# spdes/chirpgp

Measured on AMD Instinct MI355X. Metric: filter+smoother trial-steps/s (batch x T / wall), higher is better.
Workload: dtype f64; 1 GPU; C2: discrete EKF+EKS (demos/ekfs_mle.py model); d=4, T=10000, batch_per_gpu=1000, global_batch=1000, parallelism=trials sharded x1

## Files before the change

### chirpgp_amd/csrc/cgp_mfma4.hpp

```cpp
#pragma once
#include "cgp_coop4.hpp"

namespace cgp {


CGP_DEV double mfma4(double a, double b, double c) { return __builtin_amdgcn_mfma_f64_4x4x4f64(a, b, c, 0, 0, 0); }

constexpr int kCheckedChunks = 16;

struct Ekf4MfmaConst {
    double M0, M1, M2, M3, rho, ang;
    double Hr, Xi, Sig;
    double kc, ks, kj, kk;
    double SigHq, c0;
    double kcr, ksr, kja;
    double angm;
    double pa, pb, pA0, pB0, m1, m2;
    CGP_DEV void fold() { kcr = kc * rho; ksr = ks * rho; kja = kj * ang; angm = (kc != 0.0 || ks != 0.0) ? ang : 0.0; }
    CGP_DEV void fold_e1(int r, int q) {
        fold();
        angm = q == 0 ? ang : (q == 1 ? -ang : 0.0);
        pa = q < 2 ? rho : 0.0;
        pb = q == 0 ? -rho : (q == 1 ? rho : 0.0);
        pA0 = q == 2 ? M0 : (q == 3 ? M3 : 0.0);
        pB0 = q == 2 ? M1 : (q == 3 ? M2 : 0.0);
        m1 = r == q ? 1.0 : 0.0;
        m2 = r == (q ^ 1) ? 1.0 : 0.0;
    }
    template <bool E1> CGP_DEV void load(const HarmonicLCD<1>& model, const FilterIO& io, int64_t trial, int r, int q) {
        M0 = model.M[0]; M1 = model.M[1]; M2 = model.M[2]; M3 = model.M[3];
        rho = model.rho;
        ang = (model.dt * kTwoPi) * model.fs;
        Hr = io.H[trial * io.H_stride + r];
        Xi = io.Xi[trial * io.Xi_stride];
        Sig = lane_sigma_entry(model, r, q);
        const double mq = model.q;
        SigHq = (q == 1) ? mq : 0.0;
        c0 = mq + Xi;
        kc = ((q == 0 && r == 0) || (q == 1 && r == 1)) ? 1.0 : 0.0;
        ks = (q == 0 && r == 1) ? -1.0 : ((q == 1 && r == 0) ? 1.0 : 0.0);
        kj = (r == 2 && q == 0) ? -1.0 : ((r == 2 && q == 1) ? 1.0 : 0.0);
        kk = (q == 2) ? (r == 2 ? M0 : (r == 3 ? M1 : 0.0)) : ((q == 3) ? (r == 2 ? M2 : (r == 3 ? M3 : 0.0)) : 0.0);
        if constexpr (E1) fold_e1(r, q);
        else fold();
    }
};
struct Ekf4State {
    double P, ur, uq;
    CGP_DEV double u2() const { return dpp_f64<kQuadBcast2>(uq); }
    CGP_DEV double u2_replicated() const { return row_bcast_f64<2>(uq); }
    template <bool E1> CGP_DEV void load(const FilterIO& io, int64_t trial, int r, int q) {
        const double* __restrict__ m0p = io.m0 + trial * io.m0_stride;
        ur = E1 ? 0.0 : m0p[r]; uq = m0p[q];
        P = coop4_load_sym_entry(io.P0 + trial * io.P0_stride, r, q);
    }
};

template <int E1 = 0, bool GAPS = false>
CGP_DEV void ekf4_mfma_finish_j(const Ekf4MfmaConst& K, double y, double A, double B2, double kjd, Ekf4State& x, double& S, double& innov) {
    double J0T, f_r, f_q;
    if constexpr (E1 != 0) {
        f_q = fma(A, x.uq, B2 * dpp_f64<kQuadSwap1>(x.uq));
        J0T = fma(K.m1, A, K.m2 * B2);
        f_r = 0.0;
    } else {
        J0T = A;
        f_r = mfma4(J0T, x.ur, 0.0); f_q = mfma4(x.ur, J0T, 0.0);
    }
    const double RJT = fma(kjd, dpp_f64<kQuadSwap1>(f_q), J0T);
    double Pp, PHr, PHq;
    if constexpr (E1 != 0) {
        auto bcast1 = [](double v) { if constexpr (E1 == 2) return row_bcast_f64<1>(v); else return dpp_f64<kQuadBcast1>(v); };
        const double Q = mfma4(x.P, RJT, 0.0);
        const double Pa = bcast1(Q);
        PHq = mfma4(Pa, RJT, K.SigHq);
        Pp = mfma4(RJT, Q, K.Sig);
        PHr = bcast1(Pp);
        if constexpr (E1 == 1) {
            const double a = dpp_f64<kQuadBcast1>(RJT);
            S = mfma4(a, Pa, K.c0);
        } else {
            S = bcast1(PHq) + K.Xi;
        }
        innov = y - bcast1(f_q);
    } else {
        const double Q = mfma4(x.P, RJT, 0.0);
        Pp = mfma4(RJT, Q, K.Sig);
        PHr = mfma4(Pp, K.Hr, 0.0);
        PHq = mfma4(K.Hr, Pp, 0.0);
        S = mfma4(K.Hr, PHr, K.Xi);
        innov = y - mfma4(K.Hr, f_r, 0.0);
    }
    double rS = rcp_nr1(S), dy = innov;
    if constexpr (GAPS) {
        const bool gap = is_missing(y);
        rS = gap ? 0.0 : rS;
        dy = gap ? 0.0 : innov;
    }
    x.P = fma(-(PHr * rS), PHq, Pp);
    const double g = rS * dy;
    if constexpr (E1 == 0) x.ur = fma(PHr, g, f_r);
    x.uq = fma(PHq, g, f_q);
}
template <int E1 = 0, bool GAPS = false>
CGP_DEV void ekf4_mfma_finish(const Ekf4MfmaConst& K, double y, double c1, double s1, double dsp, Ekf4State& x, double& S, double& innov) {
    if constexpr (E1 != 0) {
        ekf4_mfma_finish_j<E1, GAPS>(K, y, fma(K.pa, c1, K.pA0), fma(K.pb, s1, K.pB0), K.kja * dsp, x, S, innov);
    } else {
        const double J0T = fma(K.kcr, c1, fma(K.ksr, s1, K.kk));
        ekf4_mfma_finish_j<E1, GAPS>(K, y, J0T, 0.0, K.kja * dsp, x, S, innov);
    }
}

template <int E1 = 0, bool GAPS = false>
CGP_DEV void ekf4_mfma_step_wide(const Ekf4MfmaConst& K, const WideRegs& W, double y, Ekf4State& x, double& S, double& innov, bool& bad) {
    double sp, dsp, s1, c1;
    bool ok1, ok2;
    softplus_pair_any(W, x.u2(), sp, dsp, ok1);
    fast_sincos_spec(W, K.ang * sp, s1, c1, ok2);
    bad = bad || !(ok1 && ok2);
    ekf4_mfma_finish<E1, GAPS>(K, y, c1, s1, dsp, x, S, innov);
}

template <int E1 = 0, bool GAPS = false>
CGP_DEV void ekf4_mfma_step_checked(const Ekf4MfmaConst& K, double y, Ekf4State& x, double& S, double& innov) {
    double sp, dsp, s1, c1;
    softplus_pair_uniform(x.u2(), sp, dsp);
    fast_sincos_uniform(K.ang * sp, s1, c1);
    ekf4_mfma_finish<E1, GAPS>(K, y, c1, s1, dsp, x, S, innov);
}

struct Ekf4Anchor {
    double th, A, B;
    template <int E1 = 0>
    CGP_DEV void set(const Ekf4MfmaConst& K, double sp, double c1, double s1) {
        th = K.angm * sp;
        if constexpr (E1 != 0) {
            A = fma(K.pa, c1, K.pA0);
            B = fma(K.pb, s1, K.pB0);
        } else {
            A = fma(K.kcr, c1, fma(K.ksr, s1, K.kk));
            B = fma(K.ksr, c1, -(K.kcr * s1));
        }
    }
};

template <int E1 = 0>
CGP_DEV void ekf4_anchor(const Ekf4MfmaConst& K, double u2, Ekf4Anchor& a) {
    double sp, dsp, s1, c1;
    softplus_pair_uniform(u2, sp, dsp);
    fast_sincos_uniform(K.ang * sp, s1, c1);
    a.template set<E1>(K, sp, c1, s1);
}

constexpr unsigned kIncrementBound = 0x3F780000u;
constexpr int kRegCommon = 0, kRegHigh = 1, kRegLow = 2, kRegAny = 3, kRegMid = 4;
struct Ekf4Verdict {
    unsigned u = 0u, umin = 0xFFFFFFFFu, d = 0u;
    int di = 0;
    bool any_bad = false;
    unsigned uabs = 0u;
    template <int REG = kRegCommon> CGP_DEV bool state_in_regime() const {
        if constexpr (REG == kRegAny) return !any_bad;
        if constexpr (REG == kRegMid) return uabs < 0x40000000u;
        if constexpr (REG == kRegLow) return umin >= 0xBFF80000u && u <= 0xC085DFFFu;
        constexpr unsigned lo = REG == kRegHigh ? 0x40140000u : 0x3FF80000u;
        return u <= 0x4085DFFFu && umin >= lo;
    }
    template <int REG = kRegCommon> CGP_DEV unsigned code() const {
        const bool state = __builtin_amdgcn_ballot_w64(!state_in_regime<REG>()) != 0;
        const bool jump = __builtin_amdgcn_ballot_w64((d & 0x7FFFFFFFu) >= kIncrementBound || ((unsigned)di & 0x7FFFFFFFu) >= kIncrementBound) != 0;
        return (state ? 1u : 0u) | (jump ? 2u : 0u);
    }
    template <int REG = kRegCommon> CGP_DEV unsigned long long uncommon() const {
        return __builtin_amdgcn_ballot_w64(!state_in_regime<REG>()) |
               __builtin_amdgcn_ballot_w64((d & 0x7FFFFFFFu) >= kIncrementBound || ((unsigned)di & 0x7FFFFFFFu) >= kIncrementBound);
    }
};
template <int E1, int REG = kRegCommon>
CGP_DEV void ekf4_mfma_step_spec1(const Ekf4MfmaConst& K, const SpecRegs& R, const SpecRegsHigh& RH, double y, Ekf4State& x, Ekf4Anchor& a,
                                  double& S, double& innov, Ekf4Verdict& verdict, const SpecRegsMid* RM = nullptr, const WideRegs* RW = nullptr) {
    const double u2 = (E1 == 2) ? x.u2_replicated() : x.u2();
    constexpr bool HIGH = REG == kRegHigh, LOW = REG == kRegLow, ANY = REG == kRegAny, MID = REG == kRegMid;
    double d, jfac;
    if constexpr (MID) {
        double ga, hj;
        softplus_mid_polys(*RM, u2, ga, hj);
        d = ga + fma(0.5 * K.angm, u2, -a.th);
        jfac = fma(u2, hj, 0.5 * K.kja);
    } else if constexpr (ANY) {
        double sp, dspf; bool ok;
        if (RW) softplus_pair_any(*RW, u2, sp, dspf, ok);
        else softplus_pair_any(u2, sp, dspf, ok);
        verdict.any_bad = verdict.any_bad || !ok;
        d = fma(K.angm, sp, -a.th);
        jfac = K.kja * dspf;
    } else {
        const double t = HIGH ? exp_neg_high(R, RH, u2) : exp_neg_lean1(R, LOW ? -u2 : u2);
        const double lin = LOW ? -a.th : fma(K.angm, u2, -a.th);
        double qa, dsp;
        if constexpr (HIGH) softplus_tail_high(RH, t, qa, dsp);
        else softplus_tail_lean(R, t, qa, dsp);
        d = fma(qa, t, lin);
        jfac = HIGH ? dsp : LOW ? (K.kja * t) * dsp : K.kja * dsp;
    }
    const double d2 = d * d;
    const double tau = d * fma(d2, R.c4, 0.5);
    const double sn = d * fma(d2, R.s3, 1.0);
    const double A1 = fma(tau, a.B, a.A);
    const double B = fma(-sn, A1, a.B);
    const double A = fma(tau, B, A1);
    const unsigned hx = (unsigned)__double2hiint(u2), hd = (unsigned)__double2hiint(d);
    if constexpr (MID) {
        const unsigned ha = hx & 0x7FFFFFFFu;
        verdict.uabs = verdict.uabs > ha ? verdict.uabs : ha;
    } else if constexpr (!ANY) {
        verdict.u = verdict.u > hx ? verdict.u : hx;
        verdict.umin = verdict.umin < hx ? verdict.umin : hx;
    }
    verdict.d = verdict.d > hd ? verdict.d : hd;
    verdict.di = verdict.di > (int)hd ? verdict.di : (int)hd;
    a.th += d; a.A = A; a.B = B;
    ekf4_mfma_finish_j<E1>(K, y, A, B, jfac, x, S, innov);
}

constexpr int kEkf4Unroll = 4;
constexpr int kEkf4FastGroups = 4;

#ifdef CGP_EKF4_KERNELS
template <bool E1>
CGP_DEV void ekf4_mfma_trial(const FilterIO& io, const ModelArgs& ma) {
    const int lane = threadIdx.x;
    const int r = lane >> 4, q = lane & 3;
    const FilterSpan span = filter_span(io, blockIdx.x);
    using Seg = SegRecord<4>;
    const int64_t trial = span.trial;

    HarmonicLCD<1> model;
    model.setup(ma.params + trial * ma.param_stride, ma.dt, ma.model_id);
    Ekf4MfmaConst K;
    K.template load<E1>(model, io, trial, r, q);
    Ekf4State x;
    x.template load<E1>(io, trial, r, q);
    const double* __restrict__ ys = io.record(trial);
    Tile4FilterOut out;
    out.init(io, trial, lane);
    const unsigned p_off = out.offP, m_off = out.offm;
    const bool nll_final = (io.flags & CGP_NLL_FINAL_ONLY) != 0;
    double* __restrict__ nll = (io.nll && !nll_final) ? io.nll + trial * io.T : nullptr;
    const bool want_nll = io.nll != nullptr;

    SpecRegs R;
    R.init(K.angm);
    SpecRegsHigh RH;
    RH.init(K.angm, K.kja);
    constexpr int kParkStride = 2;
    __shared__ double2 park[64 * kParkStride];
    __shared__ double ybuf[64 + 16];
    __shared__ double parkS[64], parkI[64];
    double cum = 0.0;
    int checked_left = 0, spec_off = 0, jump_streak = 0, spec_score = -4;
    unsigned n_high = 0, n_common = 0, n_redo = 0, n_checked = 0, n_high_left = 0, n_wide = 0, n_low = 0, n_mid = 0;
    Ekf4Anchor anchor_live;
    int anchor_age = -1;
    const int64_t Te = span.t_end;
    double ynext = (span.t_begin + lane < Te) ? ys[span.t_begin + lane] : 0.0;
    for (int64_t t0 = span.t_begin; t0 < Te; t0 += 64) {
        wave_lds_fence();
        const bool burn = t0 < span.t_out;
        const OobWindow Pw = out.P_window(burn), mw = out.m_window(burn);
        if (span.state && span.seg > 0 && t0 == span.t_out) {
            Seg::put_mean(span.state, Seg::kJunction, lane < 4, lane, x.uq);
            Seg::put_cov(span.state, Seg::kJunction, ((lane >> 2) & 3) == 0, r, q, x.P);
        }
        double ychunk = ynext;
        asm volatile("" : "+v"(ychunk));
        ynext = (t0 + 64 + lane < Te) ? ys[t0 + 64 + lane] : 0.0;
        const int nsteps = (Te - t0 < 64) ? (int)(Te - t0) : 64;
        const Ekf4State x0 = x;
        const unsigned hx0 = (unsigned)__builtin_amdgcn_readfirstlane(__double2hiint(x.u2()));
        const bool low = !nll_final && hx0 - 0xBFFC0000u <= 0xC085DFFFu - 0xBFFC0000u;
        const bool mid = !nll_final && (hx0 & 0x7FFFFFFFu) < 0x3FF80000u;
        const bool edge = !nll_final && !mid && (hx0 & 0x7FFFFFFFu) < 0x3FFC0000u;
        ybuf[lane] = ychunk;
        wave_lds_fence();
        Ekf4Anchor anchor0, anchor_end;
        const bool spec_allowed = spec_off == 0;
        if (!spec_allowed) anchor0 = anchor_live;
        else if (anchor_age < 0 || anchor_age >= 4) { ekf4_anchor<E1 ? 2 : 0>(K, x.u2(), anchor0); anchor_age = 0; }
        else anchor0 = anchor_live;
        auto chunk = [&](auto reg_c) {
            constexpr int REG = decltype(reg_c)::value;
            SpecRegsMid RM;
            if constexpr (REG == kRegMid) RM.init(K.angm, K.kja);
            WideRegs RW;
            if constexpr (REG == kRegAny) RW.init();
            Ekf4Anchor anchor = anchor0;
            Ekf4Verdict verdict;
            auto one = [&](int slot, unsigned k, double y) {
                double S, innov;
                ekf4_mfma_step_spec1<E1 ? 2 : 0, REG>(K, R, RH, y, x, anchor, S, innov, verdict, &RM, REG == kRegAny ? &RW : nullptr);
                park[(slot + k) * kParkStride] = make_double2(S, innov);
                const unsigned t = (unsigned)(t0 + slot);
                Pw.store_s(x.P, p_off + k * 128u, t * 128u);
                mw.store_s(x.uq, m_off + k * 32u, t * 32u);
            };
            int slot = 0;
            double2 ya = *reinterpret_cast<const double2*>(ybuf), yb = *reinterpret_cast<const double2*>(ybuf + 2);
            double2 yc = *reinterpret_cast<const double2*>(ybuf + 4), yd = *reinterpret_cast<const double2*>(ybuf + 6);
            for (; slot + 8 <= nsteps; slot += 8) {
                const double2 na = *reinterpret_cast<const double2*>(ybuf + slot + 8), nb = *reinterpret_cast<const double2*>(ybuf + slot + 10);
                const double2 nc = *reinterpret_cast<const double2*>(ybuf + slot + 12), nd = *reinterpret_cast<const double2*>(ybuf + slot + 14);
                one(slot, 0u, ya.x); one(slot, 1u, ya.y); one(slot, 2u, yb.x); one(slot, 3u, yb.y);
                one(slot, 4u, yc.x); one(slot, 5u, yc.y); one(slot, 6u, yd.x); one(slot, 7u, yd.y);
                ya = na; yb = nb; yc = nc; yd = nd;
            }
            for (; slot + 4 <= nsteps; slot += 4) {
                const double2 na = *reinterpret_cast<const double2*>(ybuf + slot + 4), nb = *reinterpret_cast<const double2*>(ybuf + slot + 6);
                one(slot, 0u, ya.x); one(slot, 1u, ya.y); one(slot, 2u, yb.x); one(slot, 3u, yb.y);
                ya = na; yb = nb;
            }
            for (; slot < nsteps; slot++) one(slot, 0u, readlane_f64(ychunk, slot));
            anchor_end = anchor;
            return verdict.template code<REG>();
        };
        unsigned uncommon = 1;
        int kept_reg = -1;
        const bool lean_tried = spec_allowed && (low || mid || (checked_left == 0 && !edge));
        if (lean_tried) {
            bool high = false;
            if constexpr (E1) high = !nll_final && hx0 - 0x401A0000u < 0x4085DFFFu - 0x401A0000u;
            if (low) {
                uncommon = chunk(std::integral_constant<int, kRegLow>{});
                if (uncommon == 0) n_low++;
            } else if (mid) {
                uncommon = chunk(std::integral_constant<int, kRegMid>{});
                if (uncommon == 0) n_mid++;
            } else {
                if (high) {
                    uncommon = chunk(std::integral_constant<int, kRegHigh>{});
                    if (uncommon != 0) { x = x0; n_high_left++; } else { n_high++; kept_reg = kRegHigh; }
                }
                if (uncommon != 0) {
                    uncommon = chunk(std::integral_constant<int, kRegCommon>{});
                    if (uncommon == 0) { n_common++; kept_reg = kRegCommon; }
                }
            }
        }
        if (uncommon != 0) {
            if (lean_tried) { x = x0; checked_left = (!(low || mid) && (uncommon & 1u)) ? kCheckedChunks : 1; n_redo++; }
            auto jumped = [&]() { jump_streak = jump_streak < 4 ? jump_streak + 1 : 4; if (spec_off < (1 << jump_streak)) spec_off = 1 << jump_streak; };
            auto failed = [&]() {
                spec_score = spec_score > -14 ? spec_score - 2 : -16;
                if (spec_score <= -8 && spec_off < 32) spec_off = 32;
                if (t0 == span.t_begin && spec_off < 8) spec_off = 8;
            };
            if (lean_tried) { failed(); if ((uncommon & 2u) != 0) jumped(); }
            if (spec_allowed && spec_off == 0) {
                uncommon = chunk(std::integral_constant<int, kRegAny>{});
                if (uncommon == 0) { if (!lean_tried) n_wide++; }
                else { failed(); if ((uncommon & 2u) != 0) jumped(); }
            }
        }
        if (uncommon == 0) {
            anchor_live = anchor_end; anchor_age++;
            if (jump_streak > 0) jump_streak--;
            if (spec_score < 8) spec_score++;
            if (checked_left > 0) checked_left--;
        } else {
            if (!spec_allowed) spec_off--;
            anchor_age = -1;
            x = x0;
            const bool redo = lean_tried;
            bool bad = false;
            WideRegs W;
            W.init();
            auto wide_one = [&](int slot, double y) {
                double S, innov;
                ekf4_mfma_step_wide<E1 ? 2 : 0>(K, W, y, x, S, innov, bad);
                park[slot * kParkStride] = make_double2(S, innov);
                const unsigned t = (unsigned)(t0 + slot);
                Pw.store_s(x.P, p_off, t * 128u);
                mw.store_s(x.uq, m_off, t * 32u);
            };
            int wslot = 0;
            for (; wslot + 4 <= nsteps; wslot += 4) {
                const double2 ya = *reinterpret_cast<const double2*>(ybuf + wslot), yb = *reinterpret_cast<const double2*>(ybuf + wslot + 2);
                wide_one(wslot, ya.x); wide_one(wslot + 1, ya.y); wide_one(wslot + 2, yb.x); wide_one(wslot + 3, yb.y);
            }
            for (; wslot < nsteps; wslot++) wide_one(wslot, readlane_f64(ychunk, wslot));
            if (__builtin_amdgcn_ballot_w64(bad) != 0) {
                x = x0;
                for (int slot = 0; slot < nsteps; slot++) {
                    double S, innov;
                    ekf4_mfma_step_checked<E1 ? 2 : 0>(K, readlane_f64(ychunk, slot), x, S, innov);
                    park[slot * kParkStride] = make_double2(S, innov);
                    const unsigned t = (unsigned)(t0 + slot);
                    Pw.store_s(x.P, p_off, t * 128u);
                    mw.store_s(x.uq, m_off, t * 32u);
                }
                if (!redo) n_checked++;
            } else if (!redo) n_wide++;
            if (checked_left > 0) checked_left--;
        }
        if (want_nll && !burn) {
            wave_lds_fence();
            const double2 si = park[(lane < nsteps ? lane : 0) * kParkStride];
            cum = nll_flush_wave(si.x, si.y, lane, nsteps, cum, nll ? nll + t0 : nullptr);
        }
        if (kept_reg >= 0 && checked_left == 0 && spec_off == 0 && t0 >= span.t_out) {
            auto fast_run = [&](auto reg_c) {
                constexpr int REG = decltype(reg_c)::value;
                for (;;) {
                    const int64_t t1 = t0 + 64;
                    if (t1 + 64 > Te) break;
                    const unsigned hx1 = (unsigned)__builtin_amdgcn_readfirstlane(__double2hiint(x.u2()));
                    const bool low1 = !nll_final && hx1 - 0xBFFC0000u <= 0xC085DFFFu - 0xBFFC0000u;
                    const bool mid1 = !nll_final && (hx1 & 0x7FFFFFFFu) < 0x3FF80000u;
                    const bool edge1 = !nll_final && !mid1 && (hx1 & 0x7FFFFFFFu) < 0x3FFC0000u;
                    bool high1 = false;
                    if constexpr (E1) high1 = !nll_final && hx1 - 0x401A0000u < 0x4085DFFFu - 0x401A0000u;
                    if (low1 || mid1 || edge1 || high1 != (REG == kRegHigh)) break;
                    wave_lds_fence();
                    double ychunk = ynext;
                    asm volatile("" : "+v"(ychunk));
                    ynext = (t1 + 64 + lane < Te) ? ys[t1 + 64 + lane] : 0.0;
                    const Ekf4State x1 = x;
                    ybuf[lane] = ychunk;
                    wave_lds_fence();
                    const bool reanchor = anchor_age >= 4;
                    Ekf4Anchor anchor;
                    if (reanchor) ekf4_anchor<E1 ? 2 : 0>(K, x.u2(), anchor);
                    else anchor = anchor_live;
                    Ekf4Verdict verdict;
                    auto one = [&](int slot, unsigned k, double y) {
                        double S, innov;
                        ekf4_mfma_step_spec1<E1 ? 2 : 0, REG>(K, R, RH, y, x, anchor, S, innov, verdict);
                        parkS[slot + k] = S; parkI[slot + k] = innov;
                        const unsigned t = (unsigned)(t1 + slot);
                        out.wP.store_s(x.P, p_off + k * 128u, t * 128u);
                        out.wm.store_s(x.uq, m_off + k * 32u, t * 32u);
                    };
                    double2 ya = *reinterpret_cast<const double2*>(ybuf), yb = *reinterpret_cast<const double2*>(ybuf + 2);
                    double2 yc = *reinterpret_cast<const double2*>(ybuf + 4), yd = *reinterpret_cast<const double2*>(ybuf + 6);
                    auto group8 = [&](int slot) {
                        const double2 na = *reinterpret_cast<const double2*>(ybuf + slot + 8), nb = *reinterpret_cast<const double2*>(ybuf + slot + 10);
                        const double2 nc = *reinterpret_cast<const double2*>(ybuf + slot + 12), nd = *reinterpret_cast<const double2*>(ybuf + slot + 14);
                        one(slot, 0u, ya.x); one(slot, 1u, ya.y); one(slot, 2u, yb.x); one(slot, 3u, yb.y);
                        one(slot, 4u, yc.x); one(slot, 5u, yc.y); one(slot, 6u, yd.x); one(slot, 7u, yd.y);
                        ya = na; yb = nb; yc = nc; yd = nd;
                    };
#pragma unroll 1
                    for (int slot = 0; slot < 64; slot += 8 * kEkf4FastGroups) {
#pragma unroll
                        for (int g = 0; g < kEkf4FastGroups; g++) group8(slot + 8 * g);
                    }
                    if (verdict.template code<REG>() != 0) { x = x1; ynext = ychunk; break; }
                    t0 = t1;
                    anchor_live = anchor; anchor_age = reanchor ? 1 : anchor_age + 1;
                    if (jump_streak > 0) jump_streak--;
                    if (spec_score < 8) spec_score++;
                    if constexpr (REG == kRegHigh) n_high++;
                    else n_common++;
                    if (want_nll) {
                        wave_lds_fence();
                        const double2 si = make_double2(parkS[lane], parkI[lane]);
                        cum = nll_flush_wave(si.x, si.y, lane, 64, cum, nll ? nll + t1 : nullptr);
                    }
                }
            };
            if (E1 && kept_reg == kRegHigh) { if constexpr (E1) fast_run(std::integral_constant<int, kRegHigh>{}); }
            else fast_run(std::integral_constant<int, kRegCommon>{});
        }
    }
    if (span.state) {
        Seg::put_mean(span.state, Seg::kEnd, lane < 4, lane, x.uq);
        Seg::put_cov(span.state, Seg::kEnd, ((lane >> 2) & 3) == 0, r, q, x.P);
        Seg::put_nll(span.state, lane, cum);
    } else if (lane == 0 && io.nll && nll_final) io.nll[trial] = cum;
    if (io.counters && lane == 0) {
        atomicAdd(io.counters + 0, (unsigned long long)n_high); atomicAdd(io.counters + 1, (unsigned long long)n_common);
        atomicAdd(io.counters + 2, (unsigned long long)n_redo); atomicAdd(io.counters + 3, (unsigned long long)n_checked);
        atomicAdd(io.counters + 4, (unsigned long long)n_high_left); atomicAdd(io.counters + 5, (unsigned long long)n_wide);
        atomicAdd(io.counters + 6, (unsigned long long)n_low); atomicAdd(io.counters + 7, (unsigned long long)n_mid);
    }
}

template <bool E1>
CGP_DEV void kf4_mfma_trial(const FilterIO& io, const ModelArgs& ma) {
    const int lane = threadIdx.x;
    const int r = lane >> 4, q = lane & 3;
    const int64_t trial = blockIdx.x;
    const double* __restrict__ prm = ma.params + trial * ma.param_stride;
    const double JT = prm[q * 4 + r];
    const double Sig = prm[16 + r * 4 + q];
    const double* __restrict__ Hp = io.H + trial * io.H_stride;
    const double Hr = Hp[r];
    const double Xi = io.Xi[trial * io.Xi_stride];

    const double* __restrict__ m0p = io.m0 + trial * io.m0_stride;
    double ur = m0p[r], uq = m0p[q];
    double P = coop4_load_sym_entry(io.P0 + trial * io.P0_stride, r, q);

    const int64_t T = io.T;
    const double* __restrict__ ys = io.record(trial);
    Tile4FilterOut out;
    out.init(io, trial, lane);

    __shared__ double2 park[64];
    __shared__ double ybuf[64 + 8];
    double cum = 0.0;
    double ynext = (lane < T) ? ys[lane] : 0.0;
    for (int64_t t0 = 0; t0 < T; t0 += 64) {
        double ychunk = ynext;
        asm volatile("" : "+v"(ychunk));
        ynext = (t0 + 64 + lane < T) ? ys[t0 + 64 + lane] : 0.0;
        const int nsteps = (T - t0 < 64) ? (int)(T - t0) : 64;
        wave_lds_fence();
        auto one = [&](int slot, double y) {
            const double f_r = mfma4(JT, ur, 0.0), f_q = mfma4(ur, JT, 0.0);
            const double Q = mfma4(P, JT, 0.0);
            double Pp, PHr, PHq, S, innov;
            if constexpr (E1) {
                Pp = mfma4(JT, Q, Sig);
                PHq = mfma4(Hr, Pp, 0.0);
                PHr = dpp_f64<kQuadBcast1>(Pp);
                S = dpp_f64<kQuadBcast1>(PHq) + Xi;
                innov = y - dpp_f64<kQuadBcast1>(f_q);
            } else {
                Pp = mfma4(JT, Q, Sig);
                PHr = mfma4(Pp, Hr, 0.0);
                PHq = mfma4(Hr, Pp, 0.0);
                S = mfma4(Hr, PHr, Xi);
                innov = y - mfma4(Hr, f_r, 0.0);
            }
            const double rS = rcp_nr1(S);
            P = fma(-(PHr * rS), PHq, Pp);
            const double g = rS * innov;
            ur = fma(PHr, g, f_r);
            uq = fma(PHq, g, f_q);
            park[slot] = make_double2(S, innov);
            const unsigned t = (unsigned)(t0 + slot);
            out.wP.store_s(P, out.offP, t * 128u);
            out.wm.store_s(uq, out.offm, t * 32u);
        };
        ybuf[lane] = ychunk;
        wave_lds_fence();
        int slot = 0;
        double2 ya = *reinterpret_cast<const double2*>(ybuf), yb = *reinterpret_cast<const double2*>(ybuf + 2);
        for (; slot + 4 <= nsteps; slot += 4) {
            const double2 na = *reinterpret_cast<const double2*>(ybuf + slot + 4), nb = *reinterpret_cast<const double2*>(ybuf + slot + 6);
            one(slot, ya.x); one(slot + 1, ya.y); one(slot + 2, yb.x); one(slot + 3, yb.y);
            ya = na; yb = nb;
        }
        for (; slot < nsteps; slot++) one(slot, readlane_f64(ychunk, slot));
        if (out.want_nll) cum = out.flush_nll(park, lane, nsteps, cum, t0);
    }
    out.store_nll_total(io, trial, lane, cum);
}
__global__ void __launch_bounds__(64) kf4_mfma_kernel(FilterIO io, ModelArgs ma) {
    const int64_t trial = blockIdx.x;
    if (trial >= io.B) return;
    if (h_is_e1(io.H + trial * io.H_stride)) kf4_mfma_trial<true>(io, ma);
    else kf4_mfma_trial<false>(io, ma);
}
inline int launch_kf4_mfma(const FilterIO& io, const ModelArgs& ma, hipStream_t stream) {
    if (io.B <= 0 || io.T <= 0) return CGP_OK;
    if (!mfma4_rows_fit(io.T)) return CGP_E_UNSUPPORTED;
    hipLaunchKernelGGL(kf4_mfma_kernel, dim3((unsigned)io.B), dim3(64), 0, stream, io, ma);
    return hip_rc(hipGetLastError());
}

__global__ void __launch_bounds__(64) ekf4_mfma_kernel(FilterIO io, ModelArgs ma) {
    const int64_t trial = filter_span(io, blockIdx.x).trial;
    if (trial >= io.B) return;
    if (h_is_e1(io.H + trial * io.H_stride)) ekf4_mfma_trial<true>(io, ma);
    else ekf4_mfma_trial<false>(io, ma);
}


#endif

#ifdef CGP_EKF4_GAPS_KERNELS
template <bool E1>
CGP_DEV void ekf4_gaps_trial(const FilterIO& io, const ModelArgs& ma) {
    const int lane = threadIdx.x;
    const int r = lane >> 4, q = lane & 3;
    const int64_t trial = blockIdx.x;

    HarmonicLCD<1> model;
    model.setup(ma.params + trial * ma.param_stride, ma.dt, ma.model_id);
    Ekf4MfmaConst K;
    K.template load<E1>(model, io, trial, r, q);
    Ekf4State x;
    x.template load<E1>(io, trial, r, q);
    const int64_t T = io.T;
    const double* __restrict__ ys = io.record(trial);
    Tile4FilterOut out;
    out.init(io, trial, lane);
    const unsigned p_off = out.offP, m_off = out.offm;
    WideRegs W;
    W.init();

    __shared__ double2 park[64];
    __shared__ double ybuf[64];
    double cum = 0.0;
    unsigned n_wide = 0, n_checked = 0;
    double ynext = (lane < T) ? ys[lane] : 0.0;
    for (int64_t t0 = 0; t0 < T; t0 += 64) {
        wave_lds_fence();
        double ychunk = ynext;
        asm volatile("" : "+v"(ychunk));
        ynext = (t0 + 64 + lane < T) ? ys[t0 + 64 + lane] : 0.0;
        const int nsteps = (T - t0 < 64) ? (int)(T - t0) : 64;
        const Ekf4State x0 = x;
        ybuf[lane] = ychunk;
        wave_lds_fence();
        bool bad = false;
        auto wide_one = [&](int slot, double y) {
            double S, innov;
            ekf4_mfma_step_wide<E1 ? 2 : 0, true>(K, W, y, x, S, innov, bad);
            park[slot] = make_double2(S, innov);
            const unsigned t = (unsigned)(t0 + slot);
            out.wP.store_s(x.P, p_off, t * 128u);
            out.wm.store_s(x.uq, m_off, t * 32u);
        };
        int slot = 0;
        for (; slot + 4 <= nsteps; slot += 4) {
            const double2 ya = *reinterpret_cast<const double2*>(ybuf + slot), yb = *reinterpret_cast<const double2*>(ybuf + slot + 2);
            wide_one(slot, ya.x); wide_one(slot + 1, ya.y); wide_one(slot + 2, yb.x); wide_one(slot + 3, yb.y);
        }
        for (; slot < nsteps; slot++) wide_one(slot, readlane_f64(ychunk, slot));
        if (__builtin_amdgcn_ballot_w64(bad) != 0) {
            x = x0;
            for (int s = 0; s < nsteps; s++) {
                double S, innov;
                ekf4_mfma_step_checked<E1 ? 2 : 0, true>(K, readlane_f64(ychunk, s), x, S, innov);
                park[s] = make_double2(S, innov);
                const unsigned t = (unsigned)(t0 + s);
                out.wP.store_s(x.P, p_off, t * 128u);
                out.wm.store_s(x.uq, m_off, t * 32u);
            }
            n_checked++;
        } else n_wide++;
        if (out.want_nll) cum = out.template flush_nll<true>(park, lane, nsteps, cum, t0, ychunk);
    }
    out.store_nll_total(io, trial, lane, cum);
    if (io.counters && lane == 0) {
        atomicAdd(io.counters + 3, (unsigned long long)n_checked);
        atomicAdd(io.counters + 5, (unsigned long long)n_wide);
    }
}
__global__ void __launch_bounds__(64) ekf4_gaps_kernel(FilterIO io, ModelArgs ma) {
    if ((int64_t)blockIdx.x >= io.B) return;
    if (h_is_e1(io.H + (int64_t)blockIdx.x * io.H_stride)) ekf4_gaps_trial<true>(io, ma);
    else ekf4_gaps_trial<false>(io, ma);
}
inline int launch_ekf4_gaps(const FilterIO& io, const ModelArgs& ma, hipStream_t stream) {
    if (io.B <= 0 || io.T <= 0) return CGP_OK;
    if (!ekf4_mfma_fits(io) || io.segs > 1) return CGP_E_UNSUPPORTED;
    hipLaunchKernelGGL(ekf4_gaps_kernel, dim3((unsigned)io.B), dim3(64), 0, stream, io, ma);
    return hip_rc(hipGetLastError());
}
#endif


#ifdef CGP_EKF4_X4_KERNELS
template <int E1 = 0>
CGP_DEV void ekf4_mfma_step_checked_lane(const Ekf4MfmaConst& K, double y, Ekf4State& x, double& S, double& innov) {
    double sp, dsp, s1, c1;
    bool ok;
    softplus_pair_any(x.u2(), sp, dsp, ok);
    if (__builtin_expect(__builtin_amdgcn_ballot_w64(!ok) != 0, 0)) {
        double sp_n, dsp_n;
        softplus_pair(x.u2(), sp_n, dsp_n);
        sp = ok ? sp : sp_n;
        dsp = ok ? dsp : dsp_n;
    }
    fast_sincos(K.ang * sp, s1, c1);
    ekf4_mfma_finish<E1>(K, y, c1, s1, dsp, x, S, innov);
}
template <int E1 = 0>
CGP_DEV void ekf4_anchor_lane(const Ekf4MfmaConst& K, double u2, Ekf4Anchor& a) {
    double sp, dsp, s1, c1;
    softplus_pair_wide(u2, sp, dsp);
    fast_sincos(K.ang * sp, s1, c1);
    a.template set<E1>(K, sp, c1, s1);
}

template <bool DENSE, bool E1>
CGP_DEV void ekf4_mfma_x4_trials(const FilterIO& io, const ModelArgs& ma) {
    const int lane = threadIdx.x;
    const int r = lane >> 4, q = lane & 3, b = (lane >> 2) & 3;
    const int64_t first = (int64_t)blockIdx.x * 4;
    const int ntr = (io.B - first < 4) ? (int)(io.B - first) : 4;
    const int64_t trial = first + (b < ntr ? b : ntr - 1);

    HarmonicLCD<1> model;
    model.setup(ma.params + trial * ma.param_stride, ma.dt, ma.model_id);
    Ekf4MfmaConst K;
    K.template load<E1>(model, io, trial, r, q);
    Ekf4State x;
    x.template load<E1>(io, trial, r, q);

    const int64_t T = io.T;
    OobWindow mfs, Pfs;
    mfs.init(io.mfs ? io.mfs + first * T * 4 : nullptr, (int64_t)ntr * T * 32);
    Pfs.init(io.Pfs ? io.Pfs + first * T * 16 : nullptr, (int64_t)ntr * T * 128);
    const unsigned p_base = (unsigned)b * (unsigned)T * 128u + 8u * (4 * r + q);
    const unsigned m_base = (r == 0) ? (unsigned)b * (unsigned)T * 32u + 8u * q : kOobOffset;
    const bool nll_final = (io.flags & CGP_NLL_FINAL_ONLY) != 0;
    const bool want_nll = io.nll != nullptr;

    SpecRegs R;
    R.init<!DENSE>(K.angm);
    const SpecRegsHigh RH{};
    __shared__ double ych[4][64];
    __shared__ double2 park[4][64];
    double cum[4] = {0.0, 0.0, 0.0, 0.0};
    int checked_left = 0;
    for (int64_t t0 = 0; t0 < T; t0 += 64) {
        const int nsteps = (T - t0 < 64) ? (int)(T - t0) : 64;
        wave_lds_fence();
        CGP_UNROLL for (int bb = 0; bb < 4; bb++) {
            const int64_t tr = first + (bb < ntr ? bb : ntr - 1);
            ych[bb][lane] = (t0 + lane < T) ? io.record(tr)[t0 + lane] : 0.0;
        }
        wave_lds_fence();
        const Ekf4State x0 = x;
        unsigned long long uncommon = 0;
        if (checked_left == 0) {
            Ekf4Anchor anchor;
            ekf4_anchor_lane<E1 ? 1 : 0>(K, x.u2(), anchor);
            Ekf4Verdict verdict;
            auto one = [&](int slot) {
                double S, innov;
                ekf4_mfma_step_spec1<E1 ? 1 : 0>(K, R, RH, ych[b][slot], x, anchor, S, innov, verdict);
                park[b][slot] = make_double2(S, innov);
                const unsigned t = (unsigned)(t0 + slot);
                Pfs.store_s(x.P, p_base, t * 128u);
                mfs.store_s(x.uq, m_base, t * 32u);
            };
            int slot = 0;
            for (; slot + kEkf4Unroll <= nsteps; slot += kEkf4Unroll) {
                CGP_UNROLL for (int k = 0; k < kEkf4Unroll; k++) one(slot + k);
            }
            for (; slot < nsteps; slot++) one(slot);
            uncommon = verdict.uncommon();
        }
        const bool redo = uncommon != 0;
        if (checked_left > 0 || redo) {
            if (redo) { x = x0; checked_left = kCheckedChunks; }
            for (int slot = 0; slot < nsteps; slot++) {
                double S, innov;
                ekf4_mfma_step_checked_lane<E1 ? 1 : 0>(K, ych[b][slot], x, S, innov);
                park[b][slot] = make_double2(S, innov);
                const unsigned t = (unsigned)(t0 + slot);
                Pfs.store_s(x.P, p_base, t * 128u);
                mfs.store_s(x.uq, m_base, t * 32u);
            }
            checked_left--;
        }
        if (want_nll) {
            wave_lds_fence();
            CGP_UNROLL for (int bb = 0; bb < 4; bb++) {
                const double2 si = park[bb][lane < nsteps ? lane : 0];
                double* out = (!nll_final && bb < ntr) ? io.nll + (first + bb) * T + t0 : nullptr;
                cum[bb] = nll_flush_wave(si.x, si.y, lane, nsteps, cum[bb], out);
            }
        }
    }
    if (lane == 0 && io.nll && nll_final) {
        CGP_UNROLL for (int bb = 0; bb < 4; bb++) if (bb < ntr) io.nll[first + bb] = cum[bb];
    }
}

template <bool DENSE>
__global__ void __launch_bounds__(64) __attribute__((amdgpu_waves_per_eu(1, DENSE ? 2 : 1))) ekf4_mfma_x4_kernel(FilterIO io, ModelArgs ma) {
    const int64_t first = (int64_t)blockIdx.x * 4;
    if (first >= io.B) return;
    const int bq = (threadIdx.x >> 2) & 3;
    const int ntr0 = (io.B - first < 4) ? (int)(io.B - first) : 4;
    const bool e1 = h_is_e1(io.H + (first + (bq < ntr0 ? bq : ntr0 - 1)) * io.H_stride);
    if (__builtin_amdgcn_ballot_w64(!e1) == 0) ekf4_mfma_x4_trials<DENSE, true>(io, ma);
    else ekf4_mfma_x4_trials<DENSE, false>(io, ma);
}

inline int launch_ekf4_mfma_x4_impl(const FilterIO& io, const ModelArgs& ma, hipStream_t stream) {
    if (io.B <= 0 || io.T <= 0) return CGP_OK;
    if (!ekf4_mfma_x4_fits(io)) return CGP_E_UNSUPPORTED;
    if (io.B > 4096) hipLaunchKernelGGL(ekf4_mfma_x4_kernel<true>, dim3((unsigned)((io.B + 3) / 4)), dim3(64), 0, stream, io, ma);
    else hipLaunchKernelGGL(ekf4_mfma_x4_kernel<false>, dim3((unsigned)((io.B + 3) / 4)), dim3(64), 0, stream, io, ma);
    return hip_rc(hipGetLastError());
}
#endif

#ifdef CGP_EKF4_KERNELS
inline int launch_ekf4_mfma(const FilterIO& io, const ModelArgs& ma, hipStream_t stream) {
    if (io.B <= 0 || io.T <= 0) return CGP_OK;
    if (!ekf4_mfma_fits(io)) return CGP_E_UNSUPPORTED;
    hipLaunchKernelGGL(ekf4_mfma_kernel, dim3((unsigned)(io.B * (io.segs > 1 ? io.segs : 1))), dim3(64), 0, stream, io, ma);
    return hip_rc(hipGetLastError());
}

#endif

}
```

Before: 4.009 billion trial-steps/s.

## Latch per-step outputs into registers via DPP and store in coalesced batches

In the speculative fast path, each step's S/innov, covariance and mean are no longer written to LDS and stored per step. They are merged into registers with DPP row/bank masks, and P and mean are stored only every 4 or 16 steps as wider, coalesced writes. The 64-step chunk is now fully unrolled so that the latch masks become compile-time immediates, and the LDS parking arrays and one fence are dropped. This cuts per-step store instructions and LDS traffic, at the cost of more DPP ops, extra live registers and a larger unrolled body.

```diff
diff --git a/chirpgp_amd/csrc/cgp_ekf4_latch.hpp b/chirpgp_amd/csrc/cgp_ekf4_latch.hpp
--- /dev/null
+++ b/chirpgp_amd/csrc/cgp_ekf4_latch.hpp
@@ -0,0 +1,43 @@
+#pragma once
+
+#if defined(__HIPCC__) || defined(__CUDACC__)
+#define CGP_LATCH_HD __host__ __device__
+#else
+#define CGP_LATCH_HD
+#endif
+
+namespace cgp {
+namespace latch4 {
+
+struct Quads { unsigned rows, banks; };
+
+CGP_LATCH_HD constexpr int lane_r(int lane) { return lane >> 4; }
+CGP_LATCH_HD constexpr int lane_b(int lane) { return (lane >> 2) & 3; }
+CGP_LATCH_HD constexpr int lane_q(int lane) { return lane & 3; }
+CGP_LATCH_HD constexpr bool takes(Quads m, int lane) { return ((m.rows >> lane_r(lane)) & 1u) != 0 && ((m.banks >> lane_b(lane)) & 1u) != 0; }
+
+constexpr int kPfSteps = 4;
+CGP_LATCH_HD constexpr Quads pf_quads(int k) { return Quads{0xFu, 1u << (k & 3)}; }
+CGP_LATCH_HD constexpr unsigned pf_lane_offset(int lane) {
+    return (unsigned)(lane_b(lane) * 128 + (4 * lane_r(lane) + lane_q(lane)) * 8);
+}
+CGP_LATCH_HD constexpr bool pf_stores_behind(int k) { return (k & 3) == 3; }
+CGP_LATCH_HD constexpr int pf_block_first(int k) { return k - (kPfSteps - 1); }
+CGP_LATCH_HD constexpr int pf_store_group_row(int k) { return pf_block_first(k) & ~7; }
+CGP_LATCH_HD constexpr int pf_store_imm_row(int k) { return pf_block_first(k) & 7; }
+
+constexpr int kMeanSteps = 16;
+CGP_LATCH_HD constexpr Quads mean_quads(int k) { return Quads{1u << ((k >> 2) & 3), 1u << (k & 3)}; }
+CGP_LATCH_HD constexpr unsigned mean_lane_offset(int lane) {
+    return (unsigned)((4 * lane_r(lane) + lane_b(lane)) * 32 + lane_q(lane) * 8);
+}
+CGP_LATCH_HD constexpr bool mean_stores_behind(int k) { return (k & 15) == 15; }
+CGP_LATCH_HD constexpr int mean_block_first(int k) { return k - (kMeanSteps - 1); }
+CGP_LATCH_HD constexpr int mean_store_imm_row(int k) { return mean_block_first(k); }
+
+CGP_LATCH_HD constexpr int nll_register(int k) { return k & 3; }
+CGP_LATCH_HD constexpr Quads nll_quads(int k) { return Quads{1u << ((k >> 4) & 3), 1u << ((k >> 2) & 3)}; }
+CGP_LATCH_HD constexpr int nll_lane_register(int lane) { return lane_q(lane); }
+
+}
+}
diff --git a/chirpgp_amd/csrc/cgp_mfma4.hpp b/chirpgp_amd/csrc/cgp_mfma4.hpp
--- a/chirpgp_amd/csrc/cgp_mfma4.hpp
+++ b/chirpgp_amd/csrc/cgp_mfma4.hpp
@@ -1,5 +1,6 @@
 #pragma once
 #include "cgp_coop4.hpp"
+#include "cgp_ekf4_latch.hpp"
 
 namespace cgp {
 
@@ -225,7 +226,15 @@
 }
 
 constexpr int kEkf4Unroll = 4;
-constexpr int kEkf4FastGroups = 4;
+constexpr int kEkf4FastGroups = 8;
+static_assert(kEkf4FastGroups * 8 == 64, "the fast path's latch masks (cgp_ekf4_latch.hpp) are immediates of the step's index in the chunk");
+
+template <unsigned ROWS, unsigned BANKS> CGP_DEV double latch_quads_f64(double old, double x) {
+    const int lo = __builtin_amdgcn_update_dpp(__double2loint(old), __double2loint(x), 0xE4, ROWS, BANKS, false);
+    const int hi = __builtin_amdgcn_update_dpp(__double2hiint(old), __double2hiint(x), 0xE4, ROWS, BANKS, false);
+    return __hiloint2double(hi, lo);
+}
+template <int J> using step_c = std::integral_constant<int, J>;
 
 #ifdef CGP_EKF4_KERNELS
 template <bool E1>
@@ -257,7 +266,6 @@
     constexpr int kParkStride = 2;
     __shared__ double2 park[64 * kParkStride];
     __shared__ double ybuf[64 + 16];
-    __shared__ double parkS[64], parkI[64];
     double cum = 0.0;
     int checked_left = 0, spec_off = 0, jump_streak = 0, spec_score = -4;
     unsigned n_high = 0, n_common = 0, n_redo = 0, n_checked = 0, n_high_left = 0, n_wide = 0, n_low = 0, n_mid = 0;
@@ -411,6 +419,9 @@
         if (kept_reg >= 0 && checked_left == 0 && spec_off == 0 && t0 >= span.t_out) {
             auto fast_run = [&](auto reg_c) {
                 constexpr int REG = decltype(reg_c)::value;
+                double stP = 0.0, stM = 0.0;
+                double lS[4] = {0.0, 0.0, 0.0, 0.0}, lI[4] = {0.0, 0.0, 0.0, 0.0};
+                const unsigned p_off4 = latch4::pf_lane_offset(lane), m_off16 = latch4::mean_lane_offset(lane);
                 for (;;) {
                     const int64_t t1 = t0 + 64;
                     if (t1 + 64 > Te) break;
@@ -421,7 +432,6 @@
                     bool high1 = false;
                     if constexpr (E1) high1 = !nll_final && hx1 - 0x401A0000u < 0x4085DFFFu - 0x401A0000u;
                     if (low1 || mid1 || edge1 || high1 != (REG == kRegHigh)) break;
-                    wave_lds_fence();
                     double ychunk = ynext;
                     asm volatile("" : "+v"(ychunk));
                     ynext = (t1 + 64 + lane < Te) ? ys[t1 + 64 + lane] : 0.0;
@@ -433,28 +443,32 @@
                     if (reanchor) ekf4_anchor<E1 ? 2 : 0>(K, x.u2(), anchor);
                     else anchor = anchor_live;
                     Ekf4Verdict verdict;
-                    auto one = [&](int slot, unsigned k, double y) {
+                    auto one = [&](auto jc, double y) {
+                        constexpr int J = decltype(jc)::value;
                         double S, innov;
                         ekf4_mfma_step_spec1<E1 ? 2 : 0, REG>(K, R, RH, y, x, anchor, S, innov, verdict);
-                        parkS[slot + k] = S; parkI[slot + k] = innov;
-                        const unsigned t = (unsigned)(t1 + slot);
-                        out.wP.store_s(x.P, p_off + k * 128u, t * 128u);
-                        out.wm.store_s(x.uq, m_off + k * 32u, t * 32u);
+                        constexpr latch4::Quads mn = latch4::nll_quads(J), mp = latch4::pf_quads(J), mm = latch4::mean_quads(J);
+                        constexpr int reg = latch4::nll_register(J);
+                        lS[reg] = latch_quads_f64<mn.rows, mn.banks>(lS[reg], S);
+                        lI[reg] = latch_quads_f64<mn.rows, mn.banks>(lI[reg], innov);
+                        stP = latch_quads_f64<mp.rows, mp.banks>(stP, x.P);
+                        if constexpr (latch4::pf_stores_behind(J))
+                            out.wP.store_s(stP, p_off4 + (unsigned)latch4::pf_store_imm_row(J) * 128u, (unsigned)(t1 + latch4::pf_store_group_row(J)) * 128u);
+                        stM = latch_quads_f64<mm.rows, mm.banks>(stM, x.uq);
+                        if constexpr (latch4::mean_stores_behind(J)) out.wm.store_s(stM, m_off16 + (unsigned)latch4::mean_store_imm_row(J) * 32u, (unsigned)t1 * 32u);
                     };
                     double2 ya = *reinterpret_cast<const double2*>(ybuf), yb = *reinterpret_cast<const double2*>(ybuf + 2);
                     double2 yc = *reinterpret_cast<const double2*>(ybuf + 4), yd = *reinterpret_cast<const double2*>(ybuf + 6);
-                    auto group8 = [&](int slot) {
-                        const double2 na = *reinterpret_cast<const double2*>(ybuf + slot + 8), nb = *reinterpret_cast<const double2*>(ybuf + slot + 10);
-                        const double2 nc = *reinterpret_cast<const double2*>(ybuf + slot + 12), nd = *reinterpret_cast<const double2*>(ybuf + slot + 14);
-                        one(slot, 0u, ya.x); one(slot, 1u, ya.y); one(slot, 2u, yb.x); one(slot, 3u, yb.y);
-                        one(slot, 4u, yc.x); one(slot, 5u, yc.y); one(slot, 6u, yd.x); one(slot, 7u, yd.y);
+                    auto group8 = [&](auto gc) {
+                        constexpr int G = decltype(gc)::value * 8;
+                        const double2 na = *reinterpret_cast<const double2*>(ybuf + G + 8), nb = *reinterpret_cast<const double2*>(ybuf + G + 10);
+                        const double2 nc = *reinterpret_cast<const double2*>(ybuf + G + 12), nd = *reinterpret_cast<const double2*>(ybuf + G + 14);
+                        one(step_c<G + 0>{}, ya.x); one(step_c<G + 1>{}, ya.y); one(step_c<G + 2>{}, yb.x); one(step_c<G + 3>{}, yb.y);
+                        one(step_c<G + 4>{}, yc.x); one(step_c<G + 5>{}, yc.y); one(step_c<G + 6>{}, yd.x); one(step_c<G + 7>{}, yd.y);
                         ya = na; yb = nb; yc = nc; yd = nd;
                     };
-#pragma unroll 1
-                    for (int slot = 0; slot < 64; slot += 8 * kEkf4FastGroups) {
-#pragma unroll
-                        for (int g = 0; g < kEkf4FastGroups; g++) group8(slot + 8 * g);
-                    }
+                    group8(step_c<0>{}); group8(step_c<1>{}); group8(step_c<2>{}); group8(step_c<3>{});
+                    group8(step_c<4>{}); group8(step_c<5>{}); group8(step_c<6>{}); group8(step_c<7>{});
                     if (verdict.template code<REG>() != 0) { x = x1; ynext = ychunk; break; }
                     t0 = t1;
                     anchor_live = anchor; anchor_age = reanchor ? 1 : anchor_age + 1;
@@ -463,9 +477,8 @@
                     if constexpr (REG == kRegHigh) n_high++;
                     else n_common++;
                     if (want_nll) {
-                        wave_lds_fence();
-                        const double2 si = make_double2(parkS[lane], parkI[lane]);
-                        cum = nll_flush_wave(si.x, si.y, lane, 64, cum, nll ? nll + t1 : nullptr);
+                        auto pick = [&](const double (&v)[4]) { return q == 0 ? v[0] : q == 1 ? v[1] : q == 2 ? v[2] : v[3]; };
+                        cum = nll_flush_wave(pick(lS), pick(lI), lane, 64, cum, nll ? nll + t1 : nullptr);
                     }
                 }
             };
```

After: 4.075 billion trial-steps/s, median of 6. 1.02x the previous value.
